# Byron/rust-tracer

Measured on AMD Instinct MI355X. Metric: Mrays/sec + ms/frame, 1920x1080 20k-sphere scene, higher is better.
Workload: dtype f32; 1 GPU; 1920x1080, 21845 spheres (pyramid L8), spp 1, f32, skip traversal, 510 64x64 buckets per frame; 1 GPU, buckets rendered straight into the row-major frame; width=1920, height=1080, samples_per_pixel=1, n_spheres=21845, primary_rays=2073600, traversal=skip, parallelism=tiles/1

## Files before the change

### rust-tracer_amd/capi.py

```python
import contextlib
import ctypes as C
import os

HERE = os.path.dirname(os.path.abspath(__file__))
PRODUCT_LIB_PATH = os.path.join(HERE, "librtrace_hip.so")
TEST_LIB_PATH = os.path.join(os.path.dirname(HERE), "tests", "c", "librtrace_hip_test.so")
LIB_PATH = os.environ.get("RTRACE_HIP_LIBRARY") or PRODUCT_LIB_PATH

RT_OK, RT_ERR_INVALID_ARGUMENT, RT_ERR_INVALID_REGION, RT_ERR_NO_DEVICE, RT_ERR_HIP, RT_ERR_OUT_OF_MEMORY, RT_ERR_UNSUPPORTED = range(7)
RT_F32, RT_F64 = 0, 1
RT_TRAVERSAL_FLAT, RT_TRAVERSAL_SKIP = 0, 1
ABI_VERSION = 5
RT_QUERY_NEAREST, RT_QUERY_ANY = 0, 1
RT_MULTIHIT_CLOSEST, RT_MULTIHIT_ALL = 0, 1
RT_MULTIHIT_MAX_K = 16
RT_UNDERSAMPLE_MAX_STEP = 64
RT_NEAR_CLOSEST, RT_NEAR_ALL = 0, 1
RT_NEAR_MAX_K = 16
RT_SWEEP_NEAREST, RT_SWEEP_ANY = 0, 1

SYMBOLS = ("rt_abi_version", "rt_build_hierarchy", "rt_device_count", "rt_scene_create", "rt_scene_destroy", "rt_scene_traits", "rt_scene_setup_cost", "rt_render_tiles",
           "rt_render_tiles_device", "rt_render_frame_device", "rt_render_region", "rt_blit_tiles_device", "rt_selftest_sqrt", "rt_selftest_rcp", "rt_tiles_rgba_bytes", "rt_strerror", "rt_last_error_message",
           "rt_host_alloc", "rt_host_free", "rt_host_register", "rt_host_unregister",
           "rt_gang_create", "rt_gang_destroy", "rt_gang_size", "rt_gang_render_frame", "rt_gang_render_frames", "rt_render_tiles_stream",
# ... 207 lines not shown
 DEBUG_FAST_KERNEL, DEBUG_EXACT_COSTS, DEBUG_MULTIHIT_BUCKET, DEBUG_TIGHT_BOUNDS) = range(25)
if HAVE_TEST_HOOKS:
    lib.rt_debug_set.argtypes = [C.c_int, C.c_longlong]
    lib.rt_debug_wave_trace.argtypes = [C.c_char_p]
    lib.rt_debug_count.restype = C.c_longlong
    lib.rt_debug_count.argtypes = [C.c_int]
    lib.rt_debug_flat_filter_check.argtypes = [C.c_void_p, C.c_uint32, C.c_uint32, C.c_uint32, C.POINTER(C.c_ulonglong * 6)]
    lib.rt_debug_gang_layout.argtypes = [C.c_void_p, C.c_uint32, C.c_uint32, C.c_void_p, C.c_void_p, C.c_void_p, C.POINTER(C.c_uint64)]
    lib.rt_debug_shard_costs.argtypes = [C.c_void_p, C.POINTER(Options), C.c_void_p, C.c_uint32, C.c_uint32, C.c_void_p]
    lib.rt_debug_rccl_library.argtypes = [C.c_char_p]
    lib.rt_debug_tight_bounds.argtypes = [C.c_void_p, C.c_uint32, C.c_void_p, C.c_void_p, C.c_void_p, C.c_void_p, C.c_uint32, C.c_void_p, C.c_void_p, C.c_void_p]


def _need_hooks(what):
    if not HAVE_TEST_HOOKS:
        raise RuntimeError("%s needs the -DRT_TEST_HOOKS build of the library: set RTRACE_HIP_LIBRARY=%s before importing rust_tracer_amd "
                           "(%s is the product and has no rt_debug_* entry point)" % (what, TEST_LIB_PATH, LIB_PATH))


def debug_count(counter):
    _need_hooks("rt_debug_count")
    return lib.rt_debug_count(counter)
(DEBUG_COUNT_REGION_CALLS, DEBUG_COUNT_REGION_PASSES, DEBUG_COUNT_FILTER_PASS, DEBUG_COUNT_FILTER_VIOLATIONS, DEBUG_COUNT_PRIMARY_TESTS,
 DEBUG_COUNT_FRAME_AHEAD_PASSES, DEBUG_COUNT_TWO_RAY_LAUNCHES, DEBUG_COUNT_COOP_LAUNCHES, DEBUG_COUNT_TIGHT_VIOLATIONS) = range(9)


def debug_set(key, value=-1):
    _need_hooks("rt_debug_set")
    check(lib.rt_debug_set(key, value), "rt_debug_set")


@contextlib.contextmanager
def debug(key, value):
    debug_set(key, value)
    try:
        yield
    finally:
        debug_set(key, -1)



def flat_filter_check(scene_handle, width, height, spp):
    _need_hooks("rt_debug_flat_filter_check")
    counts = (C.c_ulonglong * 6)()
    check(lib.rt_debug_flat_filter_check(scene_handle, width, height, spp, C.byref(counts)), "rt_debug_flat_filter_check")
    return tuple(int(c) for c in counts)

# ... 57 lines not shown
```

### rust-tracer_amd/csrc/host/host_tests.cpp

```cpp
#include <cstdio>
#include <cstdlib>

#include "render.hpp"

using namespace rtrace;

static int failures = 0;
#define CHECK(cond)                                                              \
    do {                                                                         \
        if (!(cond)) { fprintf(stderr, "FAIL %s:%d: %s\n", __FILE__, __LINE__, #cond); ++failures; } \
    } while (0)

static void vec_basics()
{
    Vector v32{ 5.0, 4.0, 0.0 };
    CHECK(v32.x == 5.0);
    CHECK(v32 == v32);
    CHECK(!(v32 != v32));
    { Vector copy = v32; copy.x = 10.0; CHECK(v32.x == 5.0 && copy.x == 10.0); }
    Vector v = v32 + v32;
    CHECK(v.x == v32.x + v32.x && v.y == v32.y + v32.y && v.z == v32.z + v32.z);
    v = v32 - v32;
    CHECK(v.x == 0.0);
    v = v32 * v32;
    CHECK(v.x == v32.x * v32.x);
    v = v32.mulfed(3.0);
// ... 55 lines not shown
}

struct DummyWriter : RGBABufferWriter {
    bool begin_called = false;
    size_t write_count = 0;
    void begin(uint16_t, uint16_t) override { begin_called = true; }
    void write_rgba_buffer(const RGBABuffer &) override { write_count += 1; }
};

static void basic_rendering()
{
    int n = 0;
    if (rt_device_count(&n) != RT_OK || n < 1) { printf("SKIP basic_rendering (no GPU; the backend has no CPU fallback)\n"); return; }
    const Scene s = Scene::default_scene();
    Backend be;
    be.devices.push_back(std::make_shared<DeviceScene>(s, 0));
    ThreadPool pool(1);
    DummyWriter dw;
    Renderer::render(RenderOptions{ 64, 128, 2 }, be, dw, pool);
    CHECK(dw.begin_called);
    CHECK(dw.write_count == 2);
}

static uint32_t crc32_of(const void *data, size_t n)
{
    static uint32_t table[256];
    static bool init = false;
    if (!init) {
        for (uint32_t i = 0; i < 256; ++i) { uint32_t c = i; for (int k = 0; k < 8; ++k) c = (c & 1u) ? 0xEDB88320u ^ (c >> 1) : c >> 1; table[i] = c; }
        init = true;
    }
    uint32_t c = 0xFFFFFFFFu;
    const uint8_t *p = static_cast<const uint8_t *>(data);
    for (size_t i = 0; i < n; ++i) c = table[(c ^ p[i]) & 0xFFu] ^ (c >> 8);
    return c ^ 0xFFFFFFFFu;
}

int main(int argc, char **argv)
{
    if (argc == 3 && std::string(argv[1]) == "--hierarchy") {
        try {
            const FlatScene f = Scene::from_file(argv[2]).flatten();
            printf("%zu %zu %u %u %u\n", f.items.size() / 4, f.ranges.size() / 2, crc32_of(f.items.data(), f.items.size() * sizeof(RFloat)),
                   crc32_of(f.bounds.data(), f.bounds.size() * sizeof(RFloat)), crc32_of(f.ranges.data(), f.ranges.size() * sizeof(int32_t)));
            return 0;
        } catch (const std::exception &e) { fprintf(stderr, "%s\n", e.what()); return 2; }
    }
    vec_basics();
    vec_default_and_normalize();
    sphere_default();
    pyramid();
    image_region();
    bucket_list();
    basic_rendering();
    if (failures) { fprintf(stderr, "%d check(s) failed\n", failures); return 1; }
    printf("host_tests ok\n");
    return 0;
}
```

### rust-tracer_amd/csrc/rt_capi.hip

```cpp
#include "../../include/rtrace_hip.h"
#include "rt_debug.h"
#include "host/hierarchy.hpp"
#include "rt_kernels.hpp"
#include "rt_skip.hpp"
#include "rt_skip_fast.hpp"
#include "rt_skip_fast64.hpp"
#include "rt_skip2_fast.hpp"
#include "rt_skip2.hpp"
#include "rt_flat.hpp"
#include "rt_flat_wf.hpp"
#include "rt_flat_sc.hpp"
#include "rt_flat_f64.hpp"
#include "rt_query.hpp"
#include "rt_trace.hpp"
#include "rt_undersample.hpp"
#include "rt_multihit.hpp"
#include "rt_near.hpp"
#include "rt_sweep.hpp"
#include "rt_contacts.hpp"
#include "rt_overlap.hpp"
#include "rt_order.hpp"
#include "rt_dynamic.hpp"
#include "rt_rebuild.hpp"

// ... 130 lines not shown
struct rt_scene {
    int device = 0;
    double setup_total_ms = 0.0, setup_first_stream_ms = 0.0;
    rt_precision precision = RT_F32;
    uint32_t n_items = 0, n_bounds = 0;
    void *d_items = nullptr;
    void *d_prim = nullptr, *d_shad = nullptr;
    void *d_cprim = nullptr, *d_cshad = nullptr;
    void *d_xprim = nullptr, *d_xshad = nullptr, *d_xcprim = nullptr, *d_xcshad = nullptr, *d_xown = nullptr;
    rt::FilterConsts fc{};
    void *d_fc = nullptr;
    uint32_t n_nodes = 0, n_fnodes = 0;
    std::vector<rt::RawNode<float>> raw_given;
    double fc_rc = 0.0;
    std::mutex tight_mu;
    bool tight_tried = false;
    int tight_by_rule = 0;
    std::atomic<bool> tight_ready{ false };
    void *d_tight = nullptr, *d_tprim = nullptr, *d_tshad = nullptr, *d_txprim = nullptr, *d_txshad = nullptr;
    uint32_t n_tight = 0;
    bool fused = false;
    void *d_coop_prim = nullptr, *d_coop_shad = nullptr;
    rt::CoopView coop{};
    void *d_fprim = nullptr, *d_fprim_rr = nullptr, *d_fshad = nullptr;
    uint32_t n_padded = 0;
    std::vector<unsigned char> h_items;
    std::mutex flat_mu;
    bool flat_ready = false;
    void *d_f64_pf = nullptr, *d_f64_sf = nullptr, *d_f64_sg = nullptr;
    double flat_centre64[3] = { 0, 0, 0 };
    void *d_pf = nullptr, *d_pe = nullptr, *d_sg = nullptr, *d_se = nullptr;
    uint32_t flat_filter_bytes = 0, flat_shadow_bytes = 0;
    float flat_centre[3] = { 0, 0, 0 };
    double light[3] = { 0, 0, 0 }, eye[3] = { 0, 0, 0 };
    std::mutex mu;
    std::vector<std::unique_ptr<Context>> pool;
    struct Order { rt::BlockDesc *dev_order = nullptr; uint32_t n_order = 0; uint32_t *dev_wg = nullptr; uint32_t n_wg = 0; uint64_t *dev_holes = nullptr; uint32_t n_holes = 0;
                   hipEvent_t e0[3] = { nullptr, nullptr, nullptr }, e1[3] = { nullptr, nullptr, nullptr }; int issued = 0, harvested = 0, good = 0; float best_ms = 1e30f; };
    struct CachedTable { std::vector<rt::TileDev> host; unsigned w = 0, h = 0, passes = 0; rt::TileDev *dev = nullptr; std::vector<Order> orders; int chosen = 0; unsigned turn = 0; bool building = false;
                         bool retrial = false;
                         void *order_arena = nullptr;
                         long long coop_key = 0;
                         hipEvent_t landed = nullptr; hipStream_t landed_on = nullptr; };
    std::vector<CachedTable> tables;
    std::vector<std::thread> builders;
    std::thread worker;
// ... 37 lines not shown
    uint8_t *d_live = nullptr;
    std::atomic<bool> live_resident{ false };
    hipEvent_t upd_ev = nullptr;
    void *d_rebuild = nullptr;
    std::mutex rebuild_mu;
    std::mutex contacts_mu;
    void *d_contacts = nullptr;
    uint32_t *d_contacts_counts = nullptr, *d_contacts_item_node = nullptr;
    uint64_t *d_contacts_offsets = nullptr, *d_contacts_sums = nullptr;
    hipEvent_t contacts_ev = nullptr;
    uint64_t *h_contacts_total = nullptr, *d_contacts_total = nullptr;
    bool contacts_recorded = false;
    std::mutex overlap_mu;
    void *d_overlap = nullptr;
    size_t overlap_cap = 0;
    uint32_t *d_overlap_counts = nullptr;
    uint64_t *d_overlap_offsets = nullptr, *d_overlap_sums = nullptr;
    hipEvent_t overlap_ev = nullptr;
    uint64_t *h_overlap_total = nullptr, *d_overlap_total = nullptr;
    bool overlap_recorded = false;
};

#include "rt_tight.hpp"

namespace {
#include "rt_capi_scene.hpp"
#include "rt_capi_dispatch.hpp"
#include "rt_capi_launch.hpp"
}

extern "C" {
#include "rt_capi_entry.hpp"
#include "rt_capi_gang.hpp"
}
```

### rust-tracer_amd/csrc/rt_capi_entry.hpp

```cpp

int rt_abi_version(void) { return RTRACE_HIP_ABI_VERSION; }

#ifdef RT_TEST_HOOKS
rt_status rt_debug_set(int key, long long value)
{
    if (key < 0 || key >= RT_DEBUG_KEYS) { snprintf(g_err, sizeof g_err, "rt_debug_set: unknown key %d", key); return RT_ERR_INVALID_ARGUMENT; }
    g_knob[key].store(value < 0 ? -1 : value, std::memory_order_relaxed);
    return RT_OK;
}

long long rt_debug_count(int counter)
{
    return counter >= 0 && counter < RT_DEBUG_COUNTERS ? g_count[counter].load(std::memory_order_relaxed) : -1;
}

rt_status rt_debug_flat_filter_check(rt_scene *s, uint32_t width, uint32_t height, uint32_t spp, unsigned long long counts[6])
{
    if (!s || !counts || !width || !height || !spp) return RT_ERR_INVALID_ARGUMENT;
    if (rt_status fst = ensure_flat(s); fst != RT_OK) return fst;
    HIP_TRY(hipSetDevice(s->device));
    unsigned long long *d = nullptr;
    HIP_TRY(hipMalloc(&d, 6 * sizeof(unsigned long long)));
    struct Free { unsigned long long *p; ~Free() { (void)hipFree(p); } } fr{ d };
    HIP_TRY(hipMemset(d, 0, 6 * sizeof(unsigned long long)));
// ... 275 lines not shown
    if (s->ahead.stream) { (void)hipStreamSynchronize(s->ahead.stream); (void)hipStreamDestroy(s->ahead.stream); }
    s->pool.clear();
    for (auto &t : s->tables) { (void)hipFree(t.dev); for (auto &od : t.orders) release_order(od); if (t.order_arena) (void)hipFree(t.order_arena); if (t.landed) (void)hipEventDestroy(t.landed); }
    if (s->dynamic) {
        s->d_shad = s->d_query_items = nullptr;
        if (s->cost_stream) (void)hipStreamSynchronize(s->cost_stream);
        if (s->d_dyn) (void)hipFree(s->d_dyn);
        if (s->upd_ev) (void)hipEventDestroy(s->upd_ev);
        if (s->d_rebuild) (void)hipFree(s->d_rebuild);
    }
    if (s->d_items) (void)hipFree(s->d_items);
    if (s->d_prim) (void)hipFree(s->d_prim);
    if (s->d_shad) (void)hipFree(s->d_shad);
    if (s->d_query_items) (void)hipFree(s->d_query_items);
    if (s->query_items_ev) (void)hipEventDestroy(s->query_items_ev);
    if (s->d_contacts) (void)hipFree(s->d_contacts);
    if (s->contacts_ev) (void)hipEventDestroy(s->contacts_ev);
    if (s->h_contacts_total) (void)hipHostFree(s->h_contacts_total);
    if (s->d_overlap) (void)hipFree(s->d_overlap);
    if (s->overlap_ev) (void)hipEventDestroy(s->overlap_ev);
    if (s->h_overlap_total) (void)hipHostFree(s->h_overlap_total);
    if (s->d_cprim) (void)hipFree(s->d_cprim);
    if (s->d_cshad) (void)hipFree(s->d_cshad);
    for (void *p : { s->d_xprim, s->d_xshad, s->d_xcprim, s->d_xcshad, s->d_xown, s->d_fc, s->d_coop_prim, s->d_coop_shad, s->d_cost_arena, s->d_tight }) if (p) (void)hipFree(p);
    if (s->cost_stream) { (void)hipStreamSynchronize(s->cost_stream); (void)hipStreamDestroy(s->cost_stream); }
    if (s->h_cost) (void)hipHostFree(s->h_cost);
    if (s->h_up) (void)hipHostFree(s->h_up);
    if (s->ahead.ev) (void)hipEventDestroy(s->ahead.ev);
    if (s->ahead.h) (void)rt_host_free(s->ahead.h);
    if (s->ahead.h_next) (void)rt_host_free(s->ahead.h_next);
    if (s->d_fprim) (void)hipFree(s->d_fprim);
    if (s->d_fprim_rr) (void)hipFree(s->d_fprim_rr);
    if (s->d_fshad) (void)hipFree(s->d_fshad);
    for (void *p : { s->d_f64_pf, s->d_f64_sf, s->d_f64_sg }) if (p) (void)hipFree(p);
    if (s->d_pf) (void)hipFree(s->d_pf);
    if (s->d_pe) (void)hipFree(s->d_pe);
    if (s->d_sg) (void)hipFree(s->d_sg);
    if (s->d_se) (void)hipFree(s->d_se);
    delete s;
    return RT_OK;
}


rt_status rt_scene_create_dynamic(int device, rt_precision precision, const void *dfs_items, uint32_t n_items, const void *light_unit, const void *eye,
                                  const void *bounds, const rt_range *ranges, uint32_t n_bounds, rt_scene **out)
{
    if (out) *out = nullptr;
// ... 2119 lines not shown
```

### rust-tracer_amd/csrc/rt_capi_launch.hpp

```cpp
int skip_variant(const rt_scene *s)
{
    int v = 1 | 2 | 4 | 16;
    if (const long long o = knob(RT_DEBUG_SKIP_VARIANT); o >= 0) v = (int)o & 23;
    if (v & 2) v |= 1;
    if (!s->fused || !(v & 2)) v &= ~4;
    if (!s->d_xprim || !(v & 2)) v &= ~16;
#ifdef RT_TEST_HOOKS
    if ((v & 3) == 3 && g_trace_on.load(std::memory_order_relaxed)) v |= 8;
#endif
    return v;
}


rt_status ensure_sample_buffers(Context *c, size_t samples, size_t esz)
{
    const size_t need = samples * esz;
    if (c->sample_cap >= need) return RT_OK;
    if (c->d_sample_gdot) HIP_TRY(hipFree(c->d_sample_gdot));
    if (c->d_sample_state) HIP_TRY(hipFree(c->d_sample_state));
    c->d_sample_gdot = nullptr; c->d_sample_state = nullptr; c->sample_cap = 0;
    HIP_TRY(hipMalloc(&c->d_sample_gdot, need));
    HIP_TRY(hipMalloc(&c->d_sample_state, samples));
    c->sample_cap = need;
    return RT_OK;
// ... 96 lines not shown
rt::Fast2Args fast2_args(const rt_scene *s, const rt::BlockList &order, unsigned w, unsigned h, unsigned spp, unsigned frame_w, void *dst)
{
    const rt::SkipView<float> sv = skip_view_of<float>(s);
    rt::Fast2Args a{};
    a.order = order.d; a.wg_first = order.wg_first;
    a.width = w; a.height = h; a.spp = spp;
    a.nb = (FUSED ? sv.n_fnodes : sv.n_nodes) * (unsigned)sizeof(rt::Node<float>);
    a.walk_prim = FUSED ? static_cast<const void *>(sv.xfprim) : static_cast<const void *>(sv.xprim);
    a.frame_w = frame_w;
    a.items = sv.items; a.own = sv.xown;
    a.eye[0] = sv.eye.x; a.eye[1] = sv.eye.y; a.eye[2] = sv.eye.z; a.light[0] = sv.light.x; a.light[1] = sv.light.y; a.light[2] = sv.light.z;
    a.walk_shad = FUSED ? static_cast<const void *>(sv.xfshad) : static_cast<const void *>(sv.xshad);
    a.exact_shad = FUSED ? static_cast<const void *>(sv.fshad) : static_cast<const void *>(sv.shad);
    a.fc = sv.fc;
    a.dst = dst;
    return a;
}

bool walks_tight(const rt_scene *s, int v, uint64_t total_px, unsigned spp)
{
    const long long tb = knob(RT_DEBUG_TIGHT_BOUNDS);
    if (tb == 0 || s->precision != RT_F32 || s->dynamic || ((v & ~8) != 19 && (v & ~8) != 23)) return false;
    if (!s->tight_ready.load(std::memory_order_acquire)) return false;
    if (tb != 2 && (s->tight_by_rule == 0 || (s->tight_by_rule == 2 && !(spp == 1 && total_px >= kTightPartialMinPx)))) return false;
    const long long k = knob(RT_DEBUG_SKIP_RAYS);
    const bool two_rays = (k < 0 ? skip2_by_default(total_px, spp, (v & 4) ? s->n_fnodes : s->n_nodes) : k == 2) && (spp == 1 || (use_split(spp) && packed_samples(spp)));
    return !two_rays;
}

template <typename T, bool COUNT, int VAR>
rt_status launch_skip_one(const rt_scene *s, Context *c, dim3 grid, hipStream_t stream, unsigned w, unsigned h, unsigned spp,
                          const rt::TileDev *d_tab, unsigned nt, uint64_t total_px, uint8_t *d_out, rt::Counters *cnt, unsigned frame_w,
                          rt::BlockList order, [[maybe_unused]] bool tight = false)
{
    bool two_rays = false;
    constexpr bool kTwoRayFlavour = !COUNT && sizeof(T) == 4 && ((VAR & 15) == 7 || (VAR & 31) == 19);
    if constexpr (kTwoRayFlavour) {
        const long long k = knob(RT_DEBUG_SKIP_RAYS);
        two_rays = k < 0 ? skip2_by_default(total_px, spp, (VAR & 4) ? s->n_fnodes : s->n_nodes) : k == 2;
        two_rays = two_rays && (spp == 1 || (use_split(spp) && packed_samples(spp))) && !tight;
    }
    constexpr bool kCoopFlavour = !COUNT && (VAR == 19 || VAR == 23 || VAR == 31);
    if (order.holes && !(kCoopFlavour && spp == 1 && !two_rays && !order.wg_first)) {
        order.d = order.plain_d; order.n = order.plain_n; order.wg_first = order.plain_wg_first; order.n_wg = order.plain_n_wg;
        order.holes = nullptr; order.n_holes = 0;
    }
    const dim3 b(rt::kBlockThreads);
    const unsigned lds = (unsigned)std::max(0ll, knob(RT_DEBUG_LDS_BYTES));
    uint32_t *no_cost = nullptr;
    std::string trace_file;
// ... 32 lines not shown
                        return RT_OK;
                    }
                }
                hipLaunchKernelGGL((rt::k_render_skip2<rt::kSkipOne, (VAR & 16) != 0, (VAR & 4) != 0>), rgrid, b2, 0, stream, skip_view_of<float>(s), w, h, spp, d_tab, nt, d_out, sb, frame_w,
                                   order.d, order.wg_first);
                return RT_OK;
            }
        }
        if constexpr (!COUNT && sizeof(T) == 4 && ((VAR & ~8) == 19 || (VAR & ~8) == 23)) {
            const long long fk = knob(RT_DEBUG_FAST_KERNEL);
            if (spp == 1 && order.d && !order.wg_first && lds == 0 && fk != 0 && (order.holes || fk == 2)) {
                rt::FastArgs fa{};
                const rt::SkipView<float> sv = skip_view_of<float>(s, tight);
                constexpr bool kFused = (VAR & 4) != 0;
                fa.order = order.d;
                fa.walk_prim = kFused ? sv.xfprim : sv.xprim;
                fa.width = w; fa.height = h; fa.nb = (kFused ? sv.n_fnodes : sv.n_nodes) * (unsigned)sizeof(rt::Node<float>); fa.frame_w = frame_w; fa.out = d_out;
                fa.eye[0] = sv.eye.x; fa.eye[1] = sv.eye.y; fa.eye[2] = sv.eye.z; fa.light[0] = sv.light.x; fa.light[1] = sv.light.y; fa.light[2] = sv.light.z;
                fa.items = sv.items; fa.own = sv.xown; fa.walk_shad = kFused ? sv.xfshad : sv.xshad; fa.exact_shad = kFused ? sv.fshad : sv.shad;
                memcpy(fa.fc, &s->fc, sizeof fa.fc);
                fa.trace = no_cost;
                g_launch_flags |= RT_LAUNCH_FAST_KERNEL;
                if (order.holes) {
                    fa.holes = order.holes; fa.n_holes = order.n_holes; fa.cv = s->coop;
                    count_event(RT_DEBUG_COUNT_COOP_LAUNCHES); g_launch_flags |= RT_LAUNCH_COOPERATIVE;
                    hipLaunchKernelGGL((rt::k_render_skip_fast_coop<(VAR & ~8), (VAR & 8) != 0>), rgrid, b, 0, stream, fa);
                } else hipLaunchKernelGGL((rt::k_render_skip_fast<(VAR & ~8), (VAR & 8) != 0>), rgrid, b, 0, stream, fa);
                return RT_OK;
            }
        }
        if constexpr (!COUNT && sizeof(T) == 8 && ((VAR & ~8) == 19 || (VAR & ~8) == 23)) {
            const long long fk = knob(RT_DEBUG_FAST_KERNEL);
            if (spp == 1 && order.d && !order.wg_first && lds == 0 && fk != 0 && (!order.holes || s->coop.fanout != 0u)) {
                rt::FastArgs64 fa{};
                const rt::SkipView<double> sv = skip_view_of<double>(s);
                constexpr bool kFused = (VAR & 4) != 0;
                fa.order = order.d;
                fa.walk_prim = kFused ? sv.xfprim : sv.xprim;
                fa.exact_prim = kFused ? sv.fprim : sv.prim;
                fa.width = w; fa.height = h; fa.nbf = (kFused ? sv.n_fnodes : sv.n_nodes) * (unsigned)sizeof(rt::FNode); fa.frame_w = frame_w; fa.out = d_out;
                fa.items = sv.items; fa.own = sv.xown;
                fa.eye[0] = sv.eye.x; fa.eye[1] = sv.eye.y; fa.eye[2] = sv.eye.z; fa.light[0] = sv.light.x; fa.light[1] = sv.light.y; fa.light[2] = sv.light.z;
                fa.walk_shad = kFused ? sv.xfshad : sv.xshad; fa.exact_shad = kFused ? sv.fshad : sv.shad;
                memcpy(fa.fc, &s->fc, sizeof fa.fc);
                fa.trace = no_cost;
                fa.holes = order.holes; fa.n_holes = order.holes ? order.n_holes : 0u; fa.cv = s->coop;
                g_launch_flags |= RT_LAUNCH_FAST_KERNEL;
                if (order.holes) { count_event(RT_DEBUG_COUNT_COOP_LAUNCHES); g_launch_flags |= RT_LAUNCH_COOPERATIVE; }
                hipLaunchKernelGGL((rt::k_render_skip_fast64_coop<(VAR & ~8), (VAR & 8) != 0>), rgrid, b, 0, stream, fa);
                return RT_OK;
            }
        }
        if constexpr (!COUNT && (VAR == 19 || VAR == 23 || VAR == 31)) {
            if (spp == 1 && order.d && order.holes && !order.wg_first) {
                count_event(RT_DEBUG_COUNT_COOP_LAUNCHES); g_launch_flags |= RT_LAUNCH_COOPERATIVE;
                hipLaunchKernelGGL((skip_kernel<T, COUNT, VAR, rt::kSkipOne, true>()), rgrid, b, lds, stream, 
                                   skip_args_of<T>(s, tight, order.d, order.wg_first, w, h, frame_w, d_out, d_tab, nt, spp, cnt, no_cost, sb, s->coop, order.holes, order.n_holes));
                return RT_OK;
            }
        }
        if (spp == 1)
            hipLaunchKernelGGL((skip_kernel<T, COUNT, VAR, rt::kSkipOne>()), rgrid, b, lds, stream, 
                               skip_args_of<T>(s, tight, order.d, order.wg_first, w, h, frame_w, d_out, d_tab, nt, spp, cnt, no_cost, sb));
        else
            hipLaunchKernelGGL((skip_kernel<T, COUNT, VAR, rt::kSkipLoop>()), rgrid, b, lds, stream, 
                               skip_args_of<T>(s, tight, order.d, order.wg_first, w, h, frame_w, d_out, d_tab, nt, spp, cnt, no_cost, sb));
        return RT_OK;
    }
    const size_t ns = (size_t)spp * spp;
    {
        rt_status bst = ensure_sample_buffers(c, ns * total_px, sizeof(T));
        if (bst != RT_OK) return bst;
    }
    sb.gdot = static_cast<T *>(c->d_sample_gdot);
    sb.state = c->d_sample_state;
    const bool packed = packed_samples(spp);
    bool done2 = false;
    if constexpr (kTwoRayFlavour) {
        if (two_rays) {
            count_event(RT_DEBUG_COUNT_TWO_RAY_LAUNCHES); g_launch_flags |= RT_LAUNCH_TWO_RAYS;
// ... 1193 lines not shown
```

### rust-tracer_amd/csrc/rt_capi_scene.hpp

```cpp

rt_status upload_words(void *d_dst, const void *h_pinned_src, size_t bytes, hipStream_t stream)
{
    void *alias = nullptr;
    HIP_TRY(hipHostGetDevicePointer(&alias, const_cast<void *>(h_pinned_src), 0));
    const size_t n = bytes / 4;
    const unsigned blocks = (unsigned)std::min<size_t>((n + 255) / 256, 2048);
    hipLaunchKernelGGL(rt::k_upload_words, dim3(std::max(1u, blocks)), dim3(256), 0, stream, static_cast<const uint32_t *>(alias), static_cast<uint32_t *>(d_dst), n);
    HIP_TRY(hipGetLastError());
    return RT_OK;
}
rt_status scene_upload(rt_scene *s, void *d_dst, const void *src, size_t bytes)
{
    const size_t need = (bytes + 255) & ~(size_t)255;
    if (s->h_up && s->up_used + need <= s->up_cap) {
        char *h = s->h_up + s->up_used;
        memcpy(h, src, bytes);
        s->up_used += need;
        return upload_words(d_dst, h, bytes, s->cost_stream);
    }
    HIP_TRY(hipMemcpyAsync(d_dst, src, bytes, hipMemcpyHostToDevice, s->cost_stream));
    return RT_OK;
}

constexpr size_t kMaxAsyncContexts = 3;
// ... 443 lines not shown
    rt_tight::Params p{};
    for (int k = 0; k < 3; ++k) { p.eye[k] = s->eye[k]; p.m0[k] = (double)s->fc.m0[k]; }
    p.rc = s->fc_rc;
    p.S = std::max(s->fc.S, (s->fc_rc + rt_tight::dist3(p.eye, p.m0)) * (1.0 + 1e-9));
    p.eta = std::max(16.0 * rt_tight::kEps, s->fc.eta);
    return p;
}

void tight_spheres_of(const rt_scene *s, const std::vector<rt::RawNode<float>> &raw, rt_tight::Result &out)
{
    std::vector<float> sph(4 * raw.size());
    std::vector<uint32_t> skip(raw.size());
    for (size_t i = 0; i < raw.size(); ++i) { sph[4 * i] = raw[i].cx; sph[4 * i + 1] = raw[i].cy; sph[4 * i + 2] = raw[i].cz; sph[4 * i + 3] = raw[i].r; skip[i] = raw[i].skip; }
    rt_tight::build(sph.data(), skip.data(), (uint32_t)raw.size(), tight_params(s), out);
}

constexpr double kTightVolumeRatio = 0.75;
constexpr uint64_t kTightPartialMinPx = 1000000u;
inline int tight_rule(const rt_tight::Result &tr, bool fused)
{
    if (tr.n_tight == 0 || !(tr.volume_ratio <= kTightVolumeRatio)) return 0;
    return (!fused || (uint64_t)tr.n_tight * 10u >= (uint64_t)tr.n_bounds * 9u) ? 1 : 2;
}
bool ensure_tight(rt_scene *s)
{
    if (s->tight_ready.load(std::memory_order_acquire)) return true;
    std::lock_guard<std::mutex> lk(s->tight_mu);
    if (s->tight_tried) return s->tight_ready.load(std::memory_order_acquire);
    s->tight_tried = true;
    if (s->precision != RT_F32 || s->dynamic || s->raw_given.empty() || !s->d_fc) return false;
    std::vector<rt::RawNode<float>> raw;
    raw.swap(s->raw_given);
    rt_tight::Result tr;
    tight_spheres_of(s, raw, tr);
    if (tr.n_tight == 0) return false;
    for (size_t i = 0; i < raw.size(); ++i)
        if (tr.tight[i]) { raw[i].cx = tr.sphere[4 * i]; raw[i].cy = tr.sphere[4 * i + 1]; raw[i].cz = tr.sphere[4 * i + 2]; raw[i].r = tr.sphere[4 * i + 3]; }
    const size_t n = raw.size(), total = n + rt::kNodePad;
    static_assert(sizeof(rt::Node<float>) == 32 && sizeof(rt::FNode) == 32 && sizeof(rt::FNodeS) == 32, "one block of 32-byte records");
    char *d = nullptr;
    if (hipMalloc(&d, 128 * total + sizeof(rt::RawNode<float>) * n) != hipSuccess) { (void)hipGetLastError(); return false; }
    rt::RawNode<float> *d_raw = reinterpret_cast<rt::RawNode<float> *>(d + 128 * total);
    hipError_t e = hipMemcpy(d_raw, raw.data(), sizeof(rt::RawNode<float>) * n, hipMemcpyHostToDevice);
    if (e == hipSuccess) {
        const rt::V3<float> eye = { (float)s->eye[0], (float)s->eye[1], (float)s->eye[2] };
        rt::Node<float> *tp = reinterpret_cast<rt::Node<float> *>(d), *ts = reinterpret_cast<rt::Node<float> *>(d + 32 * total);
        const dim3 grid((unsigned)((total + 255) / 256));
        hipLaunchKernelGGL((rt::k_build_streams<float>), grid, dim3(256), 0, s->cost_stream, d_raw, (unsigned)n, eye, false, tp, ts);
        hipLaunchKernelGGL(rt::k_build_fstreams, grid, dim3(256), 0, s->cost_stream, tp, ts, (unsigned)total, false, s->fc, reinterpret_cast<rt::FNode *>(d + 64 * total),
                           reinterpret_cast<rt::FNodeS *>(d + 96 * total), static_cast<uint32_t *>(nullptr));
        e = hipGetLastError();
        const hipError_t se = hipStreamSynchronize(s->cost_stream);
        if (e == hipSuccess) e = se;
    }
    if (e != hipSuccess) { (void)hipGetLastError(); (void)hipFree(d); return false; }
    s->d_tight = d; s->d_tprim = d; s->d_tshad = d + 32 * total; s->d_txprim = d + 64 * total; s->d_txshad = d + 96 * total;
    s->n_tight = tr.n_tight;
    s->tight_by_rule = tight_rule(tr, s->fused);
    s->tight_ready.store(true, std::memory_order_release);
    return true;
}

template <typename T>
rt_status upload_coop(rt_scene *s, const std::vector<rt::RawNode<T>> &raw)
{
    typedef typename rt::CNodeOf<T>::type Rec;
    const uint32_t n = (uint32_t)raw.size();
    if (n == 0 || n >= rt::kCoopMaxNodes) return RT_OK;
    auto next_sibling = [&](uint32_t i) { return raw[i].skip ? raw[i].skip : i + 1u; };
    std::vector<uint32_t> perm;
    perm.reserve(n);
    for (uint32_t i = 0; i < n; i = next_sibling(i)) perm.push_back(i);
    const uint32_t n_roots = (uint32_t)perm.size();
    uint32_t fanout = n_roots;
    std::vector<uint2> link(n);
    for (uint32_t j = 0; j < perm.size(); ++j) {
        const uint32_t i = perm[j];
        if (raw[i].skip == 0u) { link[j] = make_uint2(raw[i].item, 0u); continue; }
        const uint32_t first = (uint32_t)perm.size();
        for (uint32_t c = i + 1u; c < raw[i].skip; c = next_sibling(c)) perm.push_back(c);
        const uint32_t count = (uint32_t)perm.size() - first;
        if (count == 0u) return RT_OK;
        link[j] = make_uint2(first, count);
        fanout = std::max(fanout, count);
    }
    if (perm.size() != n || fanout > rt::kCoopMaxFanout) return RT_OK;
    uint32_t *d_perm = nullptr; uint2 *d_link = nullptr;
    hipError_t e = hipMalloc(&d_perm, sizeof(uint32_t) * n);
    if (e == hipSuccess) e = hipMalloc(&d_link, sizeof(uint2) * n);
    if (e == hipSuccess && scene_upload(s, d_perm, perm.data(), sizeof(uint32_t) * n) != RT_OK) e = hipErrorUnknown;
    if (e == hipSuccess && scene_upload(s, d_link, link.data(), sizeof(uint2) * n) != RT_OK) e = hipErrorUnknown;
    if (e == hipSuccess) e = hipMalloc(&s->d_coop_prim, sizeof(Rec) * n);
    if (e == hipSuccess) e = hipMalloc(&s->d_coop_shad, sizeof(Rec) * n);
    if (e == hipSuccess) {
        hipLaunchKernelGGL(rt::k_build_coop<T>, dim3((n + 255) / 256), dim3(256), 0, s->cost_stream, s->d_prim, s->d_shad, (unsigned)sizeof(rt::Node<T>), d_perm, d_link, n,
                           static_cast<Rec *>(s->d_coop_prim), static_cast<Rec *>(s->d_coop_shad));
        e = hipGetLastError();
    }
    { const hipError_t se = hipStreamSynchronize(s->cost_stream); if (e == hipSuccess) e = se; }
    if (d_perm) (void)hipFree(d_perm);
    if (d_link) (void)hipFree(d_link);
    if (e != hipSuccess) return hip_fail(e, "upload_coop", __LINE__);
    s->coop.prim = s->d_coop_prim;
    s->coop.shad = s->d_coop_shad;
    s->coop.n_roots = n_roots;
    s->coop.fanout = fanout;
    return RT_OK;
}



struct ReadLock {
    std::shared_lock<std::shared_mutex> lk;
    explicit ReadLock(rt_scene *s) { if (s && s->dynamic) lk = std::shared_lock<std::shared_mutex>(s->dyn_mu); }
};

rt_status refuse_dynamic(const rt_scene *s, const char *what)
{
    if (!s || !s->dynamic) return RT_OK;
    snprintf(g_err, sizeof g_err, "%s: a dynamic scene has no render-path data; render it with rt_render_camera (the identity camera gives rt_render_tiles' bytes)", what);
    return RT_ERR_UNSUPPORTED;
}

template <typename T>
void dynamic_topology(const std::vector<rt::RawNode<T>> &raw, uint32_t n_items, const rt_range *ranges, uint32_t n_bounds, std::vector<uint2> &topo,
                      std::vector<uint32_t> &item_node, std::vector<uint32_t> &bound_node, std::vector<rt::RefitWork> &work)
{
    constexpr uint32_t kStride = (uint32_t)sizeof(rt::Node<T>);
    topo.resize(raw.size());
    item_node.assign(n_items, 0u);
// ... 182 lines not shown
```

### rust-tracer_amd/csrc/rt_debug.h

```cpp
#ifndef RTRACE_HIP_DEBUG_H
#define RTRACE_HIP_DEBUG_H

#include "../../include/rtrace_hip.h"

#ifdef __cplusplus
extern "C" {
#endif

typedef enum rt_debug_key {
    RT_DEBUG_SKIP_VARIANT = 0,
    RT_DEBUG_BLOCK_ORDER = 1,
    RT_DEBUG_NARROW_MAX = 2,
    RT_DEBUG_PACKED_SAMPLES = 3,
    RT_DEBUG_PRINT_STEPS = 4,
    RT_DEBUG_PRINT_COSTS = 5,
    RT_DEBUG_HOST_COPY = 6,
    RT_DEBUG_COALESCE = 7,
    RT_DEBUG_LDS_BYTES = 8,
    RT_DEBUG_WG_POLICY = 9,
    RT_DEBUG_NARROW_L2 = 10,
    RT_DEBUG_FLAT_KERNELS = 11,
    RT_DEBUG_SKIP_RAYS = 12,
    RT_DEBUG_FRAME_AHEAD = 13,
    RT_DEBUG_FILTER_RO_PERCENT = 14,
// ... 2 lines not shown
    RT_DEBUG_COOP_MAX = 17,
    RT_DEBUG_COOP_LEVEL = 18,
    RT_DEBUG_COOP_REST = 19,
    RT_DEBUG_ASYNC_ORDERS = 20,
    RT_DEBUG_FAST_KERNEL = 21,
    RT_DEBUG_EXACT_COSTS = 22,
    RT_DEBUG_MULTIHIT_BUCKET = 23,
    RT_DEBUG_TIGHT_BOUNDS = 24,
    RT_DEBUG_KEYS = 25
} rt_debug_key;

rt_status rt_debug_set(int key, long long value);

typedef enum rt_debug_counter {
    RT_DEBUG_COUNT_REGION_CALLS = 0,
    RT_DEBUG_COUNT_REGION_PASSES = 1,
    RT_DEBUG_COUNT_FILTER_PASS = 2,
    RT_DEBUG_COUNT_FILTER_VIOLATIONS = 3,
    RT_DEBUG_COUNT_PRIMARY_TESTS = 4,
    RT_DEBUG_COUNT_FRAME_AHEAD_PASSES = 5,
    RT_DEBUG_COUNT_TWO_RAY_LAUNCHES = 6,
    RT_DEBUG_COUNT_COOP_LAUNCHES = 7,
    RT_DEBUG_COUNT_TIGHT_VIOLATIONS = 8,
    RT_DEBUG_COUNTERS = 9
} rt_debug_counter;
long long rt_debug_count(int counter);

rt_status rt_debug_wave_trace(const char *path);

rt_status rt_debug_flat_filter_check(rt_scene *scene, uint32_t width, uint32_t height, uint32_t spp, unsigned long long counts[6]);

rt_status rt_debug_tight_bounds(const float *dfs_items, uint32_t n_items, const float *light_unit, const float *eye, const float *bounds, const rt_range *ranges,
                                uint32_t n_bounds, float *spheres_out, uint8_t *tight_out, double consts_out[4]);

rt_status rt_debug_gang_layout(const rt_region *tiles, uint32_t n_tiles, uint32_t n_devices, uint32_t *device_of, uint32_t *px_offset,
                               uint64_t *shard_px, uint64_t *padded_px);
rt_status rt_debug_rccl_library(const char *path);
rt_status rt_debug_shard_costs(rt_scene *scene, const rt_options *options, const rt_region *tiles, uint32_t n_tiles, uint32_t n_devices, double *cost);

#ifdef __cplusplus
}
#endif
#endif
```

Baseline: 111,400 Mrays/s.

## Build cooperative BFS node copy from tight bounds and use it in cooperative launches

Adds a second cooperative (breadth-first permuted) node record set built from the tight-bounds hierarchy, and selects it for cooperative skip launches when tight bounds are in use. Previously the cooperative kernels always read the loose-bounds records even when the tight path was chosen, so they tested looser spheres. It also factors the layout builder into a validated header with host tests. The cost is extra device memory and a second build kernel when tight bounds are prepared.

```diff
diff --git a/rust-tracer_amd/capi.py b/rust-tracer_amd/capi.py
--- a/rust-tracer_amd/capi.py
+++ b/rust-tracer_amd/capi.py
@@ -253,7 +253,7 @@
     _need_hooks("rt_debug_count")
     return lib.rt_debug_count(counter)
 (DEBUG_COUNT_REGION_CALLS, DEBUG_COUNT_REGION_PASSES, DEBUG_COUNT_FILTER_PASS, DEBUG_COUNT_FILTER_VIOLATIONS, DEBUG_COUNT_PRIMARY_TESTS,
- DEBUG_COUNT_FRAME_AHEAD_PASSES, DEBUG_COUNT_TWO_RAY_LAUNCHES, DEBUG_COUNT_COOP_LAUNCHES, DEBUG_COUNT_TIGHT_VIOLATIONS) = range(9)
+ DEBUG_COUNT_FRAME_AHEAD_PASSES, DEBUG_COUNT_TWO_RAY_LAUNCHES, DEBUG_COUNT_COOP_LAUNCHES, DEBUG_COUNT_TIGHT_VIOLATIONS, DEBUG_COUNT_COOP_TIGHT_LAUNCHES) = range(10)
 
 
 def debug_set(key, value=-1):
diff --git a/rust-tracer_amd/csrc/host/host_tests.cpp b/rust-tracer_amd/csrc/host/host_tests.cpp
--- a/rust-tracer_amd/csrc/host/host_tests.cpp
+++ b/rust-tracer_amd/csrc/host/host_tests.cpp
@@ -2,6 +2,7 @@
 #include <cstdlib>
 
 #include "render.hpp"
+#include "../rt_coop_layout.hpp"
 
 using namespace rtrace;
 
@@ -103,6 +104,62 @@
     CHECK(dw.write_count == 2);
 }
 
+struct RawStub { uint32_t skip, item; };
+static void coop_stub_pyramid(std::vector<RawStub> &raw, uint32_t &next_item, unsigned level)
+{
+    if (level == 1) { raw.push_back({ 0u, next_item++ }); return; }
+    const size_t me = raw.size();
+    raw.push_back({ 0u, 0u });
+    raw.push_back({ 0u, next_item++ });
+    for (int k = 0; k < 4; ++k) coop_stub_pyramid(raw, next_item, level - 1);
+    raw[me].skip = (uint32_t)raw.size();
+}
+static void coop_layout_holds(const std::vector<RawStub> &raw, uint32_t want_roots, uint32_t want_fanout)
+{
+    rt_coop_layout::Layout lay;
+    const uint32_t n = (uint32_t)raw.size();
+    CHECK(rt_coop_layout::build(raw.data(), n, 1u << 24, 15u, lay));
+    CHECK(lay.perm.size() == n && lay.link.size() == 2 * (size_t)n && lay.n_roots == want_roots && lay.fanout == want_fanout);
+    if (lay.perm.size() != n || lay.link.size() != 2 * (size_t)n) return;
+    std::vector<uint32_t> seen(n, 0u), pos(n, 0u);
+    for (uint32_t j = 0; j < n; ++j) { CHECK(lay.perm[j] < n); if (lay.perm[j] < n) { ++seen[lay.perm[j]]; pos[lay.perm[j]] = j; } }
+    for (uint32_t i = 0; i < n; ++i) CHECK(seen[i] == 1u);
+    auto next_sibling = [&](uint32_t i) { return raw[i].skip ? raw[i].skip : i + 1u; };
+    { uint32_t j = 0; for (uint32_t i = 0; i < n; i = next_sibling(i)) CHECK(lay.perm[j++] == i); CHECK(j == want_roots); }
+    uint32_t next_first = want_roots;
+    for (uint32_t j = 0; j < n; ++j) {
+        const uint32_t i = lay.perm[j], first = lay.link[2 * (size_t)j], count = lay.link[2 * (size_t)j + 1];
+        if (raw[i].skip == 0u) { CHECK(first == raw[i].item && count == 0u); continue; }
+        CHECK(count >= 1u && count <= want_fanout && first == next_first && first + count <= n);
+        uint32_t k = 0;
+        for (uint32_t c = i + 1u; c < raw[i].skip && first + k < n; c = next_sibling(c), ++k) CHECK(lay.perm[first + k] == c && pos[c] > j);
+        CHECK(k == count);
+        next_first = first + count;
+    }
+    CHECK(next_first == n);
+}
+static void coop_layout()
+{
+    std::vector<RawStub> raw;
+    uint32_t items = 0;
+    coop_stub_pyramid(raw, items, 5);
+    CHECK(raw.size() == 426 && items == 341);
+    coop_layout_holds(raw, 1u, 5u);
+    const std::vector<RawStub> ragged = { { 0, 0 }, { 7, 0 }, { 0, 1 }, { 6, 0 }, { 0, 2 }, { 0, 3 }, { 0, 4 }, { 0, 5 } };
+    coop_layout_holds(ragged, 3u, 3u);
+    coop_layout_holds({ { 0, 0 } }, 1u, 1u);
+    rt_coop_layout::Layout lay;
+    CHECK(!rt_coop_layout::build(ragged.data(), 0u, 1u << 24, 15u, lay));
+    CHECK(!rt_coop_layout::build(ragged.data(), (uint32_t)ragged.size(), 8u, 15u, lay));
+    CHECK(!rt_coop_layout::build(ragged.data(), (uint32_t)ragged.size(), 1u << 24, 2u, lay));
+    std::vector<RawStub> wide = { { 18, 0 } };
+    for (uint32_t k = 0; k < 17; ++k) wide.push_back({ 0, k });
+    CHECK(!rt_coop_layout::build(wide.data(), (uint32_t)wide.size(), 1u << 24, 15u, lay));
+    for (const std::vector<RawStub> &bad : { std::vector<RawStub>{ { 9, 0 }, { 0, 0 } }, std::vector<RawStub>{ { 0, 0 }, { 1, 0 }, { 0, 1 } },
+                                             std::vector<RawStub>{ { 3, 0 }, { 4, 0 }, { 0, 0 }, { 0, 1 } }, std::vector<RawStub>{ { 1, 0 }, { 0, 0 } } })
+        CHECK(!rt_coop_layout::build(bad.data(), (uint32_t)bad.size(), 1u << 24, 15u, lay));
+}
+
 static uint32_t crc32_of(const void *data, size_t n)
 {
     static uint32_t table[256];
@@ -133,6 +190,7 @@
     pyramid();
     image_region();
     bucket_list();
+    coop_layout();
     basic_rendering();
     if (failures) { fprintf(stderr, "%d check(s) failed\n", failures); return 1; }
     printf("host_tests ok\n");
diff --git a/rust-tracer_amd/csrc/rt_capi.hip b/rust-tracer_amd/csrc/rt_capi.hip
--- a/rust-tracer_amd/csrc/rt_capi.hip
+++ b/rust-tracer_amd/csrc/rt_capi.hip
@@ -176,6 +176,8 @@
     bool fused = false;
     void *d_coop_prim = nullptr, *d_coop_shad = nullptr;
     rt::CoopView coop{};
+    void *d_coop_tprim = nullptr, *d_coop_tshad = nullptr;
+    rt::CoopView coop_tight{};
     void *d_fprim = nullptr, *d_fprim_rr = nullptr, *d_fshad = nullptr;
     uint32_t n_padded = 0;
     std::vector<unsigned char> h_items;
@@ -259,6 +261,7 @@
 };
 
 #include "rt_tight.hpp"
+#include "rt_coop_layout.hpp"
 
 namespace {
 #include "rt_capi_scene.hpp"
diff --git a/rust-tracer_amd/csrc/rt_capi_entry.hpp b/rust-tracer_amd/csrc/rt_capi_entry.hpp
--- a/rust-tracer_amd/csrc/rt_capi_entry.hpp
+++ b/rust-tracer_amd/csrc/rt_capi_entry.hpp
@@ -321,7 +321,7 @@
     if (s->h_overlap_total) (void)hipHostFree(s->h_overlap_total);
     if (s->d_cprim) (void)hipFree(s->d_cprim);
     if (s->d_cshad) (void)hipFree(s->d_cshad);
-    for (void *p : { s->d_xprim, s->d_xshad, s->d_xcprim, s->d_xcshad, s->d_xown, s->d_fc, s->d_coop_prim, s->d_coop_shad, s->d_cost_arena, s->d_tight }) if (p) (void)hipFree(p);
+    for (void *p : { s->d_xprim, s->d_xshad, s->d_xcprim, s->d_xcshad, s->d_xown, s->d_fc, s->d_coop_prim, s->d_coop_shad, s->d_cost_arena, s->d_tight, s->d_coop_tprim, s->d_coop_tshad }) if (p) (void)hipFree(p);
     if (s->cost_stream) { (void)hipStreamSynchronize(s->cost_stream); (void)hipStreamDestroy(s->cost_stream); }
     if (s->h_cost) (void)hipHostFree(s->h_cost);
     if (s->h_up) (void)hipHostFree(s->h_up);
diff --git a/rust-tracer_amd/csrc/rt_capi_launch.hpp b/rust-tracer_amd/csrc/rt_capi_launch.hpp
--- a/rust-tracer_amd/csrc/rt_capi_launch.hpp
+++ b/rust-tracer_amd/csrc/rt_capi_launch.hpp
@@ -142,10 +142,21 @@
     const long long tb = knob(RT_DEBUG_TIGHT_BOUNDS);
     if (tb == 0 || s->precision != RT_F32 || s->dynamic || ((v & ~8) != 19 && (v & ~8) != 23)) return false;
     if (!s->tight_ready.load(std::memory_order_acquire)) return false;
-    if (tb != 2 && (s->tight_by_rule == 0 || (s->tight_by_rule == 2 && !(spp == 1 && total_px >= kTightPartialMinPx)))) return false;
+    if (tb != 2 && tb != 3 && (s->tight_by_rule == 0 || (s->tight_by_rule == 2 && !(spp == 1 && total_px >= kTightPartialMinPx)))) return false;
     const long long k = knob(RT_DEBUG_SKIP_RAYS);
     const bool two_rays = (k < 0 ? skip2_by_default(total_px, spp, (v & 4) ? s->n_fnodes : s->n_nodes) : k == 2) && (spp == 1 || (use_split(spp) && packed_samples(spp)));
     return !two_rays;
+}
+
+rt::CoopView coop_view_of(const rt_scene *s, bool tight, bool *is_tight)
+{
+    *is_tight = tight && s->coop_tight.fanout != 0u && knob(RT_DEBUG_TIGHT_BOUNDS) != 3;
+    return *is_tight ? s->coop_tight : s->coop;
+}
+inline void note_coop_launch(bool tight_copy)
+{
+    count_event(RT_DEBUG_COUNT_COOP_LAUNCHES); g_launch_flags |= RT_LAUNCH_COOPERATIVE;
+    if (tight_copy) count_event(RT_DEBUG_COUNT_COOP_TIGHT_LAUNCHES);
 }
 
 template <typename T, bool COUNT, int VAR>
@@ -224,8 +235,9 @@
                 fa.trace = no_cost;
                 g_launch_flags |= RT_LAUNCH_FAST_KERNEL;
                 if (order.holes) {
-                    fa.holes = order.holes; fa.n_holes = order.n_holes; fa.cv = s->coop;
-                    count_event(RT_DEBUG_COUNT_COOP_LAUNCHES); g_launch_flags |= RT_LAUNCH_COOPERATIVE;
+                    bool tight_copy = false;
+                    fa.holes = order.holes; fa.n_holes = order.n_holes; fa.cv = coop_view_of(s, tight, &tight_copy);
+                    note_coop_launch(tight_copy);
                     hipLaunchKernelGGL((rt::k_render_skip_fast_coop<(VAR & ~8), (VAR & 8) != 0>), rgrid, b, 0, stream, fa);
                 } else hipLaunchKernelGGL((rt::k_render_skip_fast<(VAR & ~8), (VAR & 8) != 0>), rgrid, b, 0, stream, fa);
                 return RT_OK;
@@ -255,9 +267,11 @@
         }
         if constexpr (!COUNT && (VAR == 19 || VAR == 23 || VAR == 31)) {
             if (spp == 1 && order.d && order.holes && !order.wg_first) {
-                count_event(RT_DEBUG_COUNT_COOP_LAUNCHES); g_launch_flags |= RT_LAUNCH_COOPERATIVE;
+                bool tight_copy = false;
+                const rt::CoopView cv = coop_view_of(s, tight, &tight_copy);
+                note_coop_launch(tight_copy);
                 hipLaunchKernelGGL((skip_kernel<T, COUNT, VAR, rt::kSkipOne, true>()), rgrid, b, lds, stream, 
-                                   skip_args_of<T>(s, tight, order.d, order.wg_first, w, h, frame_w, d_out, d_tab, nt, spp, cnt, no_cost, sb, s->coop, order.holes, order.n_holes));
+                                   skip_args_of<T>(s, tight, order.d, order.wg_first, w, h, frame_w, d_out, d_tab, nt, spp, cnt, no_cost, sb, cv, order.holes, order.n_holes));
                 return RT_OK;
             }
         }
diff --git a/rust-tracer_amd/csrc/rt_capi_scene.hpp b/rust-tracer_amd/csrc/rt_capi_scene.hpp
--- a/rust-tracer_amd/csrc/rt_capi_scene.hpp
+++ b/rust-tracer_amd/csrc/rt_capi_scene.hpp
@@ -489,6 +489,8 @@
     if (tr.n_tight == 0 || !(tr.volume_ratio <= kTightVolumeRatio)) return 0;
     return (!fused || (uint64_t)tr.n_tight * 10u >= (uint64_t)tr.n_bounds * 9u) ? 1 : 2;
 }
+void upload_coop_tight(rt_scene *s, const std::vector<rt::RawNode<float>> &tight_raw);
+
 bool ensure_tight(rt_scene *s)
 {
     if (s->tight_ready.load(std::memory_order_acquire)) return true;
@@ -524,55 +526,76 @@
     s->d_tight = d; s->d_tprim = d; s->d_tshad = d + 32 * total; s->d_txprim = d + 64 * total; s->d_txshad = d + 96 * total;
     s->n_tight = tr.n_tight;
     s->tight_by_rule = tight_rule(tr, s->fused);
+    upload_coop_tight(s, raw);
     s->tight_ready.store(true, std::memory_order_release);
     return true;
 }
 
 template <typename T>
-rt_status upload_coop(rt_scene *s, const std::vector<rt::RawNode<T>> &raw)
+bool coop_layout_of(const std::vector<rt::RawNode<T>> &raw, rt_coop_layout::Layout &lay)
+{
+    return raw.size() < rt::kCoopMaxNodes && rt_coop_layout::build(raw.data(), (uint32_t)raw.size(), rt::kCoopMaxNodes, rt::kCoopMaxFanout, lay);
+}
+template <typename T>
+hipError_t coop_records(rt_scene *s, const rt_coop_layout::Layout &lay, const void *d_prim, const void *d_shad, bool in_create, void **d_cprim, void **d_cshad)
 {
     typedef typename rt::CNodeOf<T>::type Rec;
-    const uint32_t n = (uint32_t)raw.size();
-    if (n == 0 || n >= rt::kCoopMaxNodes) return RT_OK;
-    auto next_sibling = [&](uint32_t i) { return raw[i].skip ? raw[i].skip : i + 1u; };
-    std::vector<uint32_t> perm;
-    perm.reserve(n);
-    for (uint32_t i = 0; i < n; i = next_sibling(i)) perm.push_back(i);
-    const uint32_t n_roots = (uint32_t)perm.size();
-    uint32_t fanout = n_roots;
-    std::vector<uint2> link(n);
-    for (uint32_t j = 0; j < perm.size(); ++j) {
-        const uint32_t i = perm[j];
-        if (raw[i].skip == 0u) { link[j] = make_uint2(raw[i].item, 0u); continue; }
-        const uint32_t first = (uint32_t)perm.size();
-        for (uint32_t c = i + 1u; c < raw[i].skip; c = next_sibling(c)) perm.push_back(c);
-        const uint32_t count = (uint32_t)perm.size() - first;
-        if (count == 0u) return RT_OK;
-        link[j] = make_uint2(first, count);
-        fanout = std::max(fanout, count);
-    }
-    if (perm.size() != n || fanout > rt::kCoopMaxFanout) return RT_OK;
+    const uint32_t n = (uint32_t)lay.perm.size();
+    static_assert(sizeof(uint2) == 2 * sizeof(uint32_t), "Layout::link is read as uint2");
     uint32_t *d_perm = nullptr; uint2 *d_link = nullptr;
+    void *cp = nullptr, *cs = nullptr;
     hipError_t e = hipMalloc(&d_perm, sizeof(uint32_t) * n);
     if (e == hipSuccess) e = hipMalloc(&d_link, sizeof(uint2) * n);
-    if (e == hipSuccess && scene_upload(s, d_perm, perm.data(), sizeof(uint32_t) * n) != RT_OK) e = hipErrorUnknown;
-    if (e == hipSuccess && scene_upload(s, d_link, link.data(), sizeof(uint2) * n) != RT_OK) e = hipErrorUnknown;
-    if (e == hipSuccess) e = hipMalloc(&s->d_coop_prim, sizeof(Rec) * n);
-    if (e == hipSuccess) e = hipMalloc(&s->d_coop_shad, sizeof(Rec) * n);
+    if (in_create) {
+        if (e == hipSuccess && scene_upload(s, d_perm, lay.perm.data(), sizeof(uint32_t) * n) != RT_OK) e = hipErrorUnknown;
+        if (e == hipSuccess && scene_upload(s, d_link, lay.link.data(), sizeof(uint2) * n) != RT_OK) e = hipErrorUnknown;
+    } else {
+        if (e == hipSuccess) e = hipMemcpy(d_perm, lay.perm.data(), sizeof(uint32_t) * n, hipMemcpyHostToDevice);
+        if (e == hipSuccess) e = hipMemcpy(d_link, lay.link.data(), sizeof(uint2) * n, hipMemcpyHostToDevice);
+    }
+    if (e == hipSuccess) e = hipMalloc(&cp, sizeof(Rec) * n);
+    if (e == hipSuccess) e = hipMalloc(&cs, sizeof(Rec) * n);
     if (e == hipSuccess) {
-        hipLaunchKernelGGL(rt::k_build_coop<T>, dim3((n + 255) / 256), dim3(256), 0, s->cost_stream, s->d_prim, s->d_shad, (unsigned)sizeof(rt::Node<T>), d_perm, d_link, n,
-                           static_cast<Rec *>(s->d_coop_prim), static_cast<Rec *>(s->d_coop_shad));
+        hipLaunchKernelGGL(rt::k_build_coop<T>, dim3((n + 255) / 256), dim3(256), 0, s->cost_stream, d_prim, d_shad, (unsigned)sizeof(rt::Node<T>), d_perm, d_link, n,
+                           static_cast<Rec *>(cp), static_cast<Rec *>(cs));
         e = hipGetLastError();
     }
     { const hipError_t se = hipStreamSynchronize(s->cost_stream); if (e == hipSuccess) e = se; }
     if (d_perm) (void)hipFree(d_perm);
     if (d_link) (void)hipFree(d_link);
+    if (e != hipSuccess) {
+        if (cp) (void)hipFree(cp);
+        if (cs) (void)hipFree(cs);
+        return e;
+    }
+    *d_cprim = cp; *d_cshad = cs;
+    return hipSuccess;
+}
+
+template <typename T>
+rt_status upload_coop(rt_scene *s, const std::vector<rt::RawNode<T>> &raw)
+{
+    rt_coop_layout::Layout lay;
+    if (!coop_layout_of<T>(raw, lay)) return RT_OK;
+    const hipError_t e = coop_records<T>(s, lay, s->d_prim, s->d_shad, true, &s->d_coop_prim, &s->d_coop_shad);
     if (e != hipSuccess) return hip_fail(e, "upload_coop", __LINE__);
     s->coop.prim = s->d_coop_prim;
     s->coop.shad = s->d_coop_shad;
-    s->coop.n_roots = n_roots;
-    s->coop.fanout = fanout;
-    return RT_OK;
+    s->coop.n_roots = lay.n_roots;
+    s->coop.fanout = lay.fanout;
+    return RT_OK;
+}
+
+void upload_coop_tight(rt_scene *s, const std::vector<rt::RawNode<float>> &tight_raw)
+{
+    if (s->coop.fanout == 0u) return;
+    rt_coop_layout::Layout lay;
+    if (!coop_layout_of<float>(tight_raw, lay) || lay.n_roots != s->coop.n_roots || lay.fanout != s->coop.fanout) return;
+    if (coop_records<float>(s, lay, s->d_tprim, s->d_tshad, false, &s->d_coop_tprim, &s->d_coop_tshad) != hipSuccess) { (void)hipGetLastError(); return; }
+    s->coop_tight.prim = s->d_coop_tprim;
+    s->coop_tight.shad = s->d_coop_tshad;
+    s->coop_tight.n_roots = lay.n_roots;
+    s->coop_tight.fanout = lay.fanout;
 }
 
 
diff --git a/rust-tracer_amd/csrc/rt_coop_layout.hpp b/rust-tracer_amd/csrc/rt_coop_layout.hpp
--- /dev/null
+++ b/rust-tracer_amd/csrc/rt_coop_layout.hpp
@@ -0,0 +1,47 @@
+#pragma once
+#include <algorithm>
+#include <cstdint>
+#include <vector>
+
+namespace rt_coop_layout {
+
+struct Layout {
+    std::vector<uint32_t> perm;
+    std::vector<uint32_t> link;
+    uint32_t n_roots = 0;
+    uint32_t fanout = 0;
+};
+
+template <typename R>
+bool build(const R *raw, uint32_t n, uint32_t max_nodes, uint32_t max_fanout, Layout &out)
+{
+    out = Layout{};
+    if (n == 0 || n >= max_nodes) return false;
+    auto next_sibling = [&](uint32_t i) { return raw[i].skip ? raw[i].skip : i + 1u; };
+    auto well_formed = [&](uint32_t i, uint32_t end) { return raw[i].skip == 0u || (raw[i].skip > i && raw[i].skip <= end); };
+    std::vector<uint32_t> &perm = out.perm;
+    perm.reserve(n);
+    for (uint32_t i = 0; i < n; i = next_sibling(i)) {
+        if (!well_formed(i, n)) return false;
+        perm.push_back(i);
+    }
+    out.n_roots = (uint32_t)perm.size();
+    out.fanout = out.n_roots;
+    out.link.assign(2 * (size_t)n, 0u);
+    for (uint32_t j = 0; j < perm.size(); ++j) {
+        const uint32_t i = perm[j];
+        if (raw[i].skip == 0u) { out.link[2 * (size_t)j] = raw[i].item; continue; }
+        const uint32_t first = (uint32_t)perm.size(), end = raw[i].skip;
+        for (uint32_t c = i + 1u; c < end; c = next_sibling(c)) {
+            if (!well_formed(c, end) || perm.size() >= n) return false;
+            perm.push_back(c);
+        }
+        const uint32_t count = (uint32_t)perm.size() - first;
+        if (count == 0u) return false;
+        out.link[2 * (size_t)j] = first; out.link[2 * (size_t)j + 1] = count;
+        out.fanout = std::max(out.fanout, count);
+    }
+    return perm.size() == n && out.fanout <= max_fanout;
+}
+
+}
diff --git a/rust-tracer_amd/csrc/rt_debug.h b/rust-tracer_amd/csrc/rt_debug.h
--- a/rust-tracer_amd/csrc/rt_debug.h
+++ b/rust-tracer_amd/csrc/rt_debug.h
@@ -48,7 +48,8 @@
     RT_DEBUG_COUNT_TWO_RAY_LAUNCHES = 6,
     RT_DEBUG_COUNT_COOP_LAUNCHES = 7,
     RT_DEBUG_COUNT_TIGHT_VIOLATIONS = 8,
-    RT_DEBUG_COUNTERS = 9
+    RT_DEBUG_COUNT_COOP_TIGHT_LAUNCHES = 9,
+    RT_DEBUG_COUNTERS = 10
 } rt_debug_counter;
 long long rt_debug_count(int counter);
 
```

Result: slower. 110,100 Mrays/s (-1.2%).
